# seshnadathur/victor

Measured on AMD Instinct MI355X. Metric: likelihood evals/sec (40 s-bins, 100 mu, l=0,2,4), higher is better.
Workload: dtype f64

## Files before the change

victor_amd/csrc/vk_kernel_cells.h:

```cpp
#pragma once
#include "vk_kernel_fast.h"

namespace vk {

struct CellsPlan {
  int mu, w, s, betar, da, v1, sva, image_end, acc, like, total;
};

__host__ __device__ inline int cells_range_bins(int n_mu, int cpi) { return (cpi + n_mu - 2) / n_mu + 1; }

__host__ __device__ inline CellsPlan make_cells_plan(int n_mu, int n_x, int n_s, int uni_n, int nlr, int n_beta_r,
                                                     int lut_n, int with_da, int cpi, int n_like, int n_sva = 0) {
  CellsPlan p;
  int o = fast_fixed_doubles(uni_n, nlr, lut_n);
  o = (o + 1) & ~1;
  p.mu = o;    o += 2 * n_mu;
  p.w = o;     o += kMaxEll * n_mu;
  p.s = o;     o += (n_s + 1) & ~1;
  p.betar = o; o += (n_beta_r + 1) & ~1;
  p.da = o;    o += with_da ? uni_n * 4 : 0;
  p.v1 = o;    o += with_da == 1 ? 0 : uni_n * 4;
  o = (o + 1) & ~1;
  p.sva = o;   o += (n_sva + 1) & ~1;
  p.image_end = o;
  int bins = cells_range_bins(n_mu, cpi);
  if (bins > n_s) bins = n_s;
  p.acc = o;   o += kMaxEll * (bins + 1) * kWaves;
  o = (o + 1) & ~1;
  p.like = o;  o += n_like > 0 ? like_lds_doubles(n_like) : 0;
  p.total = o;
  return p;
}

template <int NLR>
__device__ __forceinline__ void stage_cells(const TheoryArgs& a, const CellsPlan& pl, double* lds, int with_da) {
  const int tid = threadIdx.x;
  for (int i = tid; i < a.n_mu; i += kBlock) {
    const double m = a.mu[i];
    lds[pl.mu + 2 * i] = m;
    lds[pl.mu + 2 * i + 1] = sqrt(1.0 - m * m);
#pragma unroll
    for (int l = 0; l < kMaxEll; ++l) lds[pl.w + l * a.n_mu + i] = (l < a.n_ell) ? a.w_ell[l * a.n_mu + i] : 0.0;
  }
  for (int j = tid; j < a.n_s; j += kBlock) lds[pl.s + j] = a.s[j];
  stage_uni_records<NLR>(a, lds);
  if (with_da) stage_da<NLR>(a, lds + pl.da);
  if (with_da != 1) for (int e = tid; e < a.uni_n * 4; e += kBlock) lds[pl.v1 + e] = a.uni_sv_v[(e >> 2) * 8 + 4 + (e & 3)];
  if (a.n_beta_r > 0)
    for (int i = tid; i < a.n_beta_r; i += kBlock) lds[pl.betar + i] = a.beta_r[i];
  if (pl.image_end > pl.sva)
    for (int e = tid; e < a.sva_doubles; e += kBlock) lds[pl.sva + e] = a.sva[e];
}

template <int NL>
__device__ __forceinline__ void finish_point_ranges(const TheoryArgs& a, long long point, double beta, double poison, double* th,
                                                    bool gather, const double* lds_beta_r) {
  const int N = a.n_ell * a.n_s;
  const double w0 = a.wsum[0], w1 = a.wsum[1], w2 = a.wsum[2];
  const bool keep_out = !a.fuse || a.want_theory;
  LikePrefetch<kLikeRowsCells> pf;
  if (a.fuse) pf.issue(a.like, beta, late_tid(), lds_beta_r);
  for (int e = late_tid(); gather && e < N; e += kBlock) {
    const int l = (e >= 2 * a.n_s) ? 2 : (e >= a.n_s ? 1 : 0), j = e - l * a.n_s;
    const int q_first = (j * a.n_mu) / a.cells_per_item, q_last = (j * a.n_mu + a.n_mu - 1) / a.cells_per_item;
    double part[8];
    load_shared_x8(partial_slot(a, point, l, j), part);
    double v = 0.0;
#pragma unroll
    for (int c = 0; c < kMaxParts; ++c) v += (c <= q_last - q_first) ? part[c] : 0.0;
    v = v - (l == 0 ? w0 : (l == 1 ? w1 : w2)) + poison;
    if (keep_out) a.out[point * (long long)N + e] = v;
    th[e] = v;
  }
  __syncthreads();
  if (a.fuse) like_point_workgroup(a.like, point, beta, th, th + like_red_off(N), pf);
}

template <int NL>
__device__ __forceinline__ void project_trip(double g, bool first, bool second, const double* w_i, int n_mu, double* acc, int lstride, int lane) {
  const double ga = first ? g : 0.0, gb = second ? g : 0.0;
  double z[NL];
#pragma unroll
  for (int l = 0; l < NL; ++l) {
    const double w = w_i[l * n_mu];
    z[l] = vkm::fold32(w * ga, w * gb);
  }
  double x;
  int l_mine;
  bool mine;
  const int row = lane >> 4;
  if (NL == 3) {
    const double u = vkm::fold16(z[0], z[1]);
    const double v = vkm::fold16(z[2], 0.0);
    const bool up = (lane & 8) != 0;
    const double keep = up ? v : u, send = up ? u : v;
    x = keep + vkm::dpp_move<0x128, 0xF, true>(send);
    l_mine = up ? 2 : (row & 1);
    mine = (lane & 7) == 0 && !(up && (row & 1));
  } else {
    x = vkm::fold16(z[0], NL == 2 ? z[NL - 1] : 0.0);
    x += vkm::dpp_move<0x128, 0xF, true>(x);
    l_mine = row & 1;
    mine = (lane & 15) == 0 && (NL == 2 || !(row & 1));
  }
  x = vkm::octet_sum(x);
  if (mine) acc[l_mine * lstride + (lane >> 5) * kWaves] += x;
}

template <int NLR, int NL, int GRID, int MODE, int SVA = 0>
__global__ __launch_bounds__(kBlock, (MODE == kModeStreaming && !SVA) || MODE == kModeKaiser ? 5 : 4) void vk_theory_cells_kernel(TheoryArgs a) {
  extern __shared__ double lds[];
  vkm::clamp_keeps_nan();
  warm_kernarg_lines<sizeof(TheoryArgs)>();
  const int N = a.n_ell * a.n_s;
  const int R = a.parts;
  const int cpi = a.cells_per_item;
  const bool xi_out = NL == 1 && a.xi_out != 0;
  const bool tail = !xi_out && (a.fuse || R > 1);
  CellsPlan pl = make_cells_plan(a.n_mu, a.n_x, a.n_s, a.uni_n, NLR, a.n_beta_r, a.uni_lut_n, mode_layout(MODE), xi_out ? 0 : cpi,
                                 tail ? N : 0, SVA ? a.sva_doubles : 0);
  pl.like = __builtin_amdgcn_readfirstlane(pl.like);
  const int tid = threadIdx.x;
  VK_STAMP(a, 0);
  if (a.image) copy_image(lds, a.image, pl.image_end);
  else stage_cells<NLR>(a, pl, lds, mode_layout(MODE));
  constexpr bool kHalf = MODE != kModeKaiser;
  const FastConsts fc = make_fast_consts<NLR>(a, kHalf, SVA ? pl.sva : 0);
  __syncthreads();
  VK_STAMP(a, 1);

  const int lane = tid & 63;
  const int wave = __builtin_amdgcn_readfirstlane(tid >> 6);
  const double* l_mu = lds + pl.mu;
  const double* l_w = lds + pl.w;
  const double* l_s = lds + pl.s;
  const int slots = xi_out ? 1 : min(cells_range_bins(a.n_mu, cpi), a.n_s) + 1;
  double* l_acc = lds + pl.acc;
  const unsigned items = (unsigned)a.n * (unsigned)R;
  const int all_cells = a.n_s * a.n_mu;

  {
    const unsigned item = blockIdx.x;
    if (item >= items) return;
    const long long point = item / (unsigned)R;
    const int q = (int)(item - (unsigned)point * (unsigned)R);
    const int c0 = q * cpi, c1 = min(c0 + cpi, all_cells);
    const int jf = (int)__umulhi((unsigned)c0, a.nmu_magic);
    const int nb = (int)__umulhi((unsigned)(c1 - 1), a.nmu_magic) - jf + 1;
    const double* row = a.params + point * VK_NPAR;
    const PointScalars ps = point_scalars(a, row);
    const FastPoint fp = make_fast_point(ps, fc, kHalf);
    constexpr int PV = MODE == kModeKaiser ? 0 : 1;
    __syncthreads();
    rebuild_point_tables<NLR, PV>(a, lds, pl.betar, pl.v1, row[VK_P_BETA], ps.av, mode_is_dispersion(MODE) ? -fp.Gk : fp.AVk,
                                  mode_has_da(MODE) ? lds + pl.da : nullptr);
    if (mode_has_da(MODE) && a.empirical && !a.vr_beta_dep) rebuild_da_emp(a, lds + pl.da, ps.av);
    for (int e = lane; e < kMaxEll * slots; e += 64) l_acc[e * kWaves + wave] = 0.0;
    __syncthreads();
    VK_STAMP(a, 2);
    for (int base = c0 + 64 * wave; base < c1; base += 64 * kWaves) {
      const int e = base + lane;
      const bool live = e < c1;
      const unsigned ec = (unsigned)(live ? e : c1 - 1);
      const int hi = xi_out ? (a.n_s == 1 ? (int)ec : (int)__umulhi(ec, a.ns_magic)) : (int)__umulhi(ec, a.nmu_magic);
      const int lo = (int)ec - hi * (xi_out ? a.n_s : a.n_mu);
      const int j = xi_out ? lo : hi;
      const int i = xi_out ? hi : lo;
      const int jj = j - jf;
      const double sj = l_s[j];
      const vk_d2 mm = *reinterpret_cast<const vk_d2*>(l_mu + 2 * i);
      const double s_perp = sj * fp.k_perp * mm.y;
      const double sperp2 = s_perp * s_perp;
      const double sperp2x = sperp2 * fp.fp2;
      const double s_par = sj * fp.k_par * mm.x;
      double g = 0.0;
      const bool inside = !mode_has_da(MODE) && !__any(!cell_in_table(fc, s_par, sperp2, a.xw_max * fabs(fp.Bk)));
      double gs = 0.0;
      if (MODE == kModeKaiser) {
        g = kaiser_value<NLR, GRID>(lds, lds + pl.da, fc, fp, ps.M, ps.Q, a.niter, a.coord_shift != 0, a.kaiser_approx != 0,
                                    a.rsd == VK_RSD_EUCLID, a.from_data != 0, s_par, sperp2);
      } else if (mode_is_dispersion(MODE)) {
        const double inv_den0 = disp_first_pass<NLR, GRID>(lds, fc, fp, a.niter, s_par, sperp2);
        for (int k = 0; k < a.n_xg; ++k) {
          const VelocityNode xw = load_node(a.xgw, k);
          gs += disp_value<NLR, GRID, MODE == kModeDispersionFromData, SVA>(lds, lds + pl.da, fc, fp, a.niter, fma(-xw.x, fp.Bk, s_par), inv_den0,
                                                                     sperp2, xw.x);
          if (xw.last != 0) {
            asm volatile("" ::: "memory");
            g = fma(xw.w, gs, g);
            gs = 0.0;
          }
        }
      } else if (inside) {
        VelocityNode nxt = load_node(a.xgw, 0);
        for (int k = 0; k < a.n_xg; ++k) {
          const VelocityNode xw = nxt;
          nxt = load_node(a.xgw, k + 1);
          double inv_sv;
          const double p = uni_point<NLR, GRID, MODE == kModeFromData, 1, 0, 0, SVA>(lds, fc, 0.0, fma(-xw.x, fp.Bk, s_par), sperp2, xw.x, fp.fa,
                                                                            sperp2x, 0u, inv_sv);
          gs = fma(inv_sv, p, gs);
          if (xw.last != 0) {
            asm volatile("" ::: "memory");
            g = fma(xw.w, gs, g);
            gs = 0.0;
          }
        }
      } else {
        VelocityNode nxt = load_node(a.xgw, 0);
        for (int k = 0; k < a.n_xg; ++k) {
          const VelocityNode xw = nxt;
          nxt = load_node(a.xgw, k + 1);
          double inv_sv;
          const double p = uni_point<NLR, GRID, MODE == kModeFromData, 1, 1, 0, SVA>(lds, fc, 0.0, fma(-xw.x, fp.Bk, s_par), sperp2, xw.x, fp.fa,
                                                                            sperp2x, 0u, inv_sv);
          gs = fma(inv_sv, p, gs);
          if (xw.last != 0) {
            asm volatile("" ::: "memory");
            g = fma(xw.w, gs, g);
            gs = 0.0;
          }
        }
      }
      if (xi_out) {
        if (live) a.out[point * (long long)all_cells + e] = g - 1.0 + ps.poison;
        continue;
      }
      const int jj0 = __builtin_amdgcn_readfirstlane(jj);
      project_trip<NL>(g, live && jj == jj0, live && jj != jj0, l_w + i, a.n_mu, l_acc + jj0 * kWaves + wave, slots * kWaves, lane);
    }
    if (xi_out) return;
    __syncthreads();
    double* th = lds + pl.like;
    for (int e = late_tid(); e < NL * nb; e += kBlock) {
      const int l = e / nb, jl = e - l * nb;
      const int j = jf + jl;
      const double* pa = l_acc + (l * slots + jl) * kWaves;
      const double sum = (pa[0] + pa[1]) + (pa[2] + pa[3]);
      if (R > 1) {
        store_shared(partial_slot(a, point, l, j) + (q - (j * a.n_mu) / cpi), sum);
      } else {
        const double v = sum - (l == 0 ? a.wsum[0] : (l == 1 ? a.wsum[1] : a.wsum[2])) + ps.poison;
        if (!a.fuse || a.want_theory) a.out[point * (long long)N + l * a.n_s + j] = v;
        if (tail) th[l * a.n_s + j] = v;
      }
    }
    VK_STAMP(a, 3);
    if (tail) {
      bool last = true;
      if (R > 1) {
        int* flag = reinterpret_cast<int*>(th + like_red_off(N) + kLikeRed + 2);
        last = point_completed(a.counters, point, (unsigned)R, flag);
      }
      VK_STAMP(a, 4);
      if (last) {
        finish_point_ranges<NL>(a, point, row[VK_P_BETA], ps.poison, th, R > 1, a.n_beta_r > 0 ? lds + pl.betar : nullptr);
        VK_STAMP(a, 5);
      }
      return;
    }
  }
}


}
```

victor_amd/csrc/victor_hip.hip:

```cpp

#include <hip/hip_runtime.h>
#include <chrono>
#include <cstddef>

#include <cmath>
#include <cstdarg>
#include <cstdio>
#include <cstdlib>
#include <cstring>
#include <limits>
#include <new>
#include <algorithm>
#include <atomic>
#include <map>
#include <string>
#include <vector>

#include "victor_hip.h"
#include "vk_host.h"
#include "vk_ledger.h"
#include "vk_kernel_cells.h"
#include "vk_kernel_fast.h"
#include "vk_kernel_generic.h"
#ifdef VK_DEV_LANES
// ... 841 lines not shown
    ctx->fast_ok = ok;
    ctx->matter_vt = t->matter_model == VK_MATTER_VELOCITY_TEMPLATE;
    ctx->vt_amp = t->vt_amp;
    ctx->matter_lb = t->matter_model == VK_MATTER_LINEAR_BIAS;
    ctx->vr_beta_dep = t->vr_beta_dep ? 1 : 0;
  }
  Uploader up;
  const size_t o_s = up.add(t->s, t->n_s), o_mu = up.add(t->mu, t->n_mu),
               o_w = up.add(t->w_ell, (size_t)t->n_ell * t->n_mu), o_x = up.add(t->x, t->n_x),
               o_wx = up.add(t->w_x, t->n_x);
  const double zero_one[2] = {0.0, 1.0};
  const size_t o_x1 = up.add(zero_one, 2);
  std::vector<double> xw_scaled(2 * ((size_t)t->n_x + 1), 0.0);
  for (int k = 0; k < t->n_x; ++k) {
    xw_scaled[2 * k] = t->x[k] * vkm::kExpScale;
    xw_scaled[2 * k + 1] = t->w_x[k];
    ctx->xw_max = std::max(ctx->xw_max, std::fabs(xw_scaled[2 * k]));
  }
  const size_t o_xws = up.add(xw_scaled.data(), xw_scaled.size());
  std::vector<double> xgw;
  {
    std::vector<char> taken(t->n_x, 0);
    for (int k0 = 0; k0 < t->n_x; ++k0) {
      if (taken[k0] || t->w_x[k0] == 0.0) continue;
      for (int k = k0; k < t->n_x; ++k)
        if (!taken[k] && t->w_x[k] == t->w_x[k0]) {
          taken[k] = 1;
          xgw.push_back(t->x[k] * vkm::kExpScale);
          xgw.push_back(0.0);
        }
      xgw.back() = t->w_x[k0];
    }
    ctx->n_xg = (int)(xgw.size() / 2);
    xgw.resize(xgw.size() + 2, 0.0);
  }
  const size_t o_xgw = up.add(xgw.data(), xgw.size());
  const size_t o_br = t->n_beta_r > 0 ? up.add(t->beta_r, t->n_beta_r) : 0;
  const size_t xi_coef_n = t->n_beta_r > 0 ? (size_t)t->n_ell_r * (t->n_beta_r - 1) * t->xi.n_int * 16
                                           : (size_t)t->n_ell_r * t->xi.n_int * 4;
  const size_t o_xik = up.add(t->xi.knots, t->xi.n_int + 1), o_xic = up.add(t->xi.coef, xi_coef_n);
  const size_t vr_coef_n = t->vr_beta_dep ? (size_t)2 * (t->n_beta_r - 1) * t->vr.n_int * 16 : (size_t)kVrVars * t->vr.n_int * 4;
  const size_t o_vrk = up.add(t->vr.knots, t->vr.n_int + 1), o_vrc = up.add(t->vr.coef, vr_coef_n);
  const bool have_vr_emp = t->vr_beta_dep && t->vr_emp;
  const size_t o_vre = have_vr_emp ? up.add(t->vr_emp, (size_t)3 * (t->n_beta_r - 1) * t->vr.n_int * 28) : 0;
  const size_t o_svk = up.add(t->sv.knots, t->sv.n_int + 1),
               o_svc = up.add(t->sv.coef, t->sv_n_mu ? 4 : (size_t)t->sv.n_int * 4);
  size_t o_svmu = 0, o_sv2d = 0, o_sva = 0;
  if (t->sv_n_mu) {
    o_svmu = up.add(t->sv_mu, t->sv_n_mu);
    o_sv2d = up.add(t->sv2d, (size_t)t->sv.n_int * (t->sv_n_mu - 1) * 16);
    if (ctx->fast_ok) {
      const int nm = t->sv_n_mu - 1;
      const double h = 1.0 / t->sv.inv_h;
      std::vector<double> blk((size_t)t->sv.n_int * nm * 16 + t->sv_n_mu);
      for (size_t e = 0; e < (size_t)t->sv.n_int * nm * 16; ++e) {
        const int pw = (int)((e >> 2) & 3);
        blk[e] = t->sv2d[e] * (pw == 0 ? 1.0 : pw == 1 ? h : pw == 2 ? h * h : h * h * h);
      }
      for (int k = 0; k < t->sv_n_mu; ++k) blk[(size_t)t->sv.n_int * nm * 16 + k] = t->sv_mu[k];
      o_sva = up.add(blk.data(), blk.size());
      ctx->sva_doubles = (int)blk.size();
    }
  }
  size_t o_usv = 0, o_uxi = 0, o_uxc = 0, o_ulut = 0, o_uk = 0, o_uvb = 0, o_uv2 = 0, o_uda = 0, o_uge = 0, o_udab = 0, o_uempb = 0;
  const bool have_lut = t->uni_n > 0 && t->uni_lut_n > 0 && t->uni_lut && t->uni_knots;
  if (have_lut) {
    std::vector<double> packed(((size_t)t->uni_lut_n + 3) / 4, 0.0);
// ... 1108 lines not shown
```

victor_amd/csrc/vk_devmath.h:

```cpp
#pragma once

#include <hip/hip_runtime.h>

namespace vkm {

template <int CTRL, int ROW_MASK, bool BOUND_CTRL = false>
__device__ __forceinline__ double dpp_move(double v) {
  int lo = __double2loint(v), hi = __double2hiint(v);
  lo = __builtin_amdgcn_update_dpp(0, lo, CTRL, ROW_MASK, 0xF, BOUND_CTRL);
  hi = __builtin_amdgcn_update_dpp(0, hi, CTRL, ROW_MASK, 0xF, BOUND_CTRL);
  return __hiloint2double(hi, lo);
}

__device__ __forceinline__ double wave_sum(double v) {
  v += dpp_move<0xB1, 0xF, true>(v);
  v += dpp_move<0x4E, 0xF, true>(v);
  v += dpp_move<0x141, 0xF, true>(v);
  v += dpp_move<0x140, 0xF, true>(v);
  v += dpp_move<0x142, 0xF, true>(v);
  v += dpp_move<0x143, 0xF, true>(v);
  const int lo = __builtin_amdgcn_readlane(__double2loint(v), 63);
  const int hi = __builtin_amdgcn_readlane(__double2hiint(v), 63);
  return __hiloint2double(hi, lo);
}
// ... 45 lines not shown
constexpr int kExpNonposTab = 256;
__device__ __forceinline__ double exp2_frac(int j) { return exp2((double)j * (1.0 / kExpNonposTab)); }

__device__ __forceinline__ double fma3(double p, double f, double c) {
  double r;
  asm("v_fma_f64 %0, %1, %2, %3" : "=v"(r) : "v"(p), "v"(f), "v"(c));
  return r;
}

__device__ __forceinline__ double exp_nonpos(double a, const double* __restrict__ tab) {
  a = fmax(a, -750.0);
  const double n = rint(a * 369.3299304675746);
  double f = fma(n, -0x1.62e42fee00000p-9, a);
  f = fma(n, -0x1.a39ef35793c76p-41, f);
  const int ni = (int)n;
  const double t = tab[ni & (kExpNonposTab - 1)];
  double p = fma3(f, 1.0 / 24.0, 1.0 / 6.0);
  p = fma(p, f, 0.5);
  p = fma(p, f, 1.0);
  p = fma(p, f, 1.0);
  return ldexp(t * p, ni >> 8);
}

__device__ __forceinline__ double fma_s(double p, double f, double c) {
  double r;
  asm("v_fma_f64 %0, %1, %2, %3" : "=v"(r) : "v"(p), "v"(f), "s"(c));
  return r;
}

__device__ __forceinline__ double recip_nr(double x) {
  const double y = __builtin_amdgcn_rcp(x);
  const double e = fma(-x, y, 1.0);
  return fma(y, e, y);
}

__device__ __forceinline__ double rsqrt_nr_x2(double x) {
  const double y = __builtin_amdgcn_rsq(x);
  const double h = x * y;
  const double w = fma(-h, y, 3.0);
  return y * w;
}

__device__ __forceinline__ double rsqrt3_x2(double x) {
  const double y = __builtin_amdgcn_rsq(x);
  const double e = fma(-(x * y), y, 1.0);
  const double p2 = fma(0.75, e, 1.0);
  return y * fma(e, p2, 2.0);
}

constexpr double kExpScale = 13.589148804608305 * 0x1p-9;
constexpr double kExpC = 709.782712893383996843;
template <int EXPT> struct ExpCfg;
template <> struct ExpCfg<0> {
  static constexpr int kBits = 8, kEntries = 256, kDoubles = 256, kDegree = 3;
  static constexpr double kMagic = 0x1.8p34;
  static constexpr double kLead = kExpC * kExpC * kExpC / 6.0;
};
template <> struct ExpCfg<1> {
  static constexpr int kBits = 6, kEntries = 64, kDoubles = 64 * 32, kDegree = 4;
  static constexpr double kMagic = 0x1.8p36;
  static constexpr double kLead = kExpC * kExpC * kExpC * kExpC / 24.0;
};
constexpr int kExpTab = ExpCfg<0>::kDoubles;

template <int EXPT>
__device__ __forceinline__ double exp_table_entry(int j) {
// ... 45 lines not shown
```

victor_amd/csrc/vk_kernel_fast.h:

```cpp
#pragma once
#include "vk_common.h"
#include "vk_kernel_like.h"

namespace vk {

typedef double vk_d2 __attribute__((ext_vector_type(2)));
constexpr int kMuRec = 6;
constexpr int kEtabOff = 0;
template <int EXPT> __host__ __device__ constexpr int recs_off() { return vkm::ExpCfg<EXPT>::kDoubles; }
__host__ __device__ constexpr int recs_off_rt(int expt) { return expt ? vkm::ExpCfg<1>::kDoubles : vkm::ExpCfg<0>::kDoubles; }

__host__ __device__ constexpr int uni_stride(int nlr) { return 4 * (2 + nlr) + 2; }
__host__ __device__ constexpr int fast_fixed_doubles(int uni_n, int nlr, int lut_n, int expt = 0) {
  return recs_off_rt(expt) + (uni_n + (lut_n > 0 ? 2 : 0)) * uni_stride(nlr) + (lut_n + 3) / 4;
}

struct FastConsts {
  double inv_h;
  double off, t_lo, n_eps;
  double inv_g;
  double rlo2, rhi2;
  int lut_off;
  double sv_a, sv_b, sv_tmax;
  double mu_lo, mu_hi, mu_inv_h;
  int sva_off, svmu_off, sv_nm;
};

__device__ __forceinline__ double vmin_f64(double a, double b) {
  double r;
  asm("v_min_f64 %0, %1, %2" : "=v"(r) : "v"(a), "v"(b));
  return r;
}
__device__ __forceinline__ double vmax_f64(double a, double b) {
  double r;
  asm("v_max_f64 %0, %1, %2" : "=v"(r) : "v"(a), "v"(b));
  return r;
}

__device__ __forceinline__ const double* lds_at(const double* base, int byte_off) {
  return reinterpret_cast<const double*>(reinterpret_cast<const char*>(base) + byte_off);
}

__device__ __forceinline__ double cubic_b128(const double* rec, double t) {
  const vk_d2 lo = *reinterpret_cast<const vk_d2*>(rec);
  const vk_d2 hi = *reinterpret_cast<const vk_d2*>(rec + 2);
  return fma(fma(fma(hi.y, t, hi.x), t, lo.y), t, lo.x);
}

template <int NLR, int EXPT = 0>
__device__ __forceinline__ FastConsts make_fast_consts(const TheoryArgs& a, bool half, int sva_off_doubles = 0) {
  FastConsts fc;
  const double sq = half ? 0.25 : 1.0;
  fc.sv_a = fc.sv_b = fc.sv_tmax = fc.mu_lo = fc.mu_hi = fc.mu_inv_h = 0.0;
  fc.sva_off = fc.svmu_off = fc.sv_nm = 0;
  if (a.sv_n_mu > 0 && a.sva_doubles > 0 && a.uni_lut_n == 0) {
    fc.sv_a = a.sv.inv_h / a.uni_inv_h;
    fc.sv_b = -a.sv.knots[0] * a.sv.inv_h;
    fc.sv_tmax = (double)a.sv.n_int * (1.0 - 0x1p-52);
    fc.sv_nm = a.sv_n_mu - 1;
    fc.mu_lo = a.sv_mu[0];
    fc.mu_hi = a.sv_mu[fc.sv_nm];
    fc.mu_inv_h = a.sv_mu_inv_h;
    fc.sva_off = sva_off_doubles * 8;
    fc.svmu_off = (sva_off_doubles + a.sv.n_int * fc.sv_nm * 16) * 8;
  }
  if (a.uni_lut_n > 0) {
    fc.inv_h = 1.0;
    fc.off = 0.0;
    fc.t_lo = a.uni_knots[0];
    fc.n_eps = a.uni_knots[a.uni_n] * (1.0 - 0x1p-52);
    fc.inv_g = a.uni_lut_inv_g;
    fc.rlo2 = sq * fc.t_lo * fc.t_lo * (1.0 + 1e-9);
    fc.rhi2 = sq * fc.n_eps * fc.n_eps * (1.0 - 1e-9);
    fc.lut_off = (recs_off<EXPT>() + (a.uni_n + 2) * uni_stride(NLR)) * 8;
  } else {
    fc.inv_h = a.uni_inv_h;
    fc.off = -a.uni_u0 * a.uni_inv_h;
    fc.t_lo = (a.vr.knots[0] - a.uni_u0) * a.uni_inv_h;
    fc.n_eps = (double)a.uni_n * (1.0 - 0x1p-52);
    fc.inv_g = 0.0;
    const double lo = fc.t_lo - fc.off, hi = fc.n_eps - fc.off;
    fc.rlo2 = sq * lo * lo * (1.0 + 1e-9);
    fc.rhi2 = sq * hi * hi * (1.0 - 1e-9);
    fc.lut_off = 0;
  }
  return fc;
}

__device__ __forceinline__ bool cell_in_table(const FastConsts& fc, double s_par, double sperp2, double xi_max) {
  const double spx = fabs(s_par) + xi_max;
  const double spn = fmax(fabs(s_par) - xi_max, 0.0);
  return (fma(spn, spn, sperp2) >= fc.rlo2) && (fma(spx, spx, sperp2) < fc.rhi2);
}

template <int NLR, int EXPT = 0>
__device__ __forceinline__ void stage_uni_records(const TheoryArgs& a, double* lds) {
  constexpr int stride = uni_stride(NLR);
  double* recs = lds + recs_off<EXPT>();
  const int tid = threadIdx.x;
  for (int e = tid; e < a.uni_n * 8; e += kBlock) recs[(e >> 3) * stride + (e & 7)] = a.uni_sv_v[e];
  if (a.n_beta_r == 0) {
    const double* src = (NLR > 1) ? a.uni_xic : a.uni_xi;
    const int per_l = a.uni_n * 4;
    for (int e = tid; e < NLR * per_l; e += kBlock) {
      const int l = e / per_l, iq = e - l * per_l;
      recs[(iq >> 2) * stride + 8 + 4 * l + (iq & 3)] = src[e];
    }
  }
  const double* etab = EXPT ? a.exp_tab_rep : a.exp_tab;
  for (int j = tid; j < vkm::ExpCfg<EXPT>::kDoubles; j += kBlock) lds[kEtabOff + j] = etab[j];
  if (a.uni_lut_n > 0) {
    for (int q = tid; q <= a.uni_n + 1; q += kBlock) {
      const double left = a.uni_knots[q < a.uni_n ? q : a.uni_n];
      recs[q * stride + stride - 2] = left;
      recs[q * stride + stride - 1] = (q < a.uni_n) ? 1.0 / (a.uni_knots[q + 1] - left) : 0.0;
      if (q >= a.uni_n)
        for (int e = 0; e < stride - 2; ++e) recs[q * stride + e] = 0.0;
    }
    unsigned short* lut = reinterpret_cast<unsigned short*>(recs + (a.uni_n + 2) * stride);
    for (int c = tid; c < a.uni_lut_n; c += kBlock) lut[c] = a.uni_lut[c];
  }
}

__device__ __forceinline__ double poly6(const double* __restrict__ c, double db) {
  double v = c[6];
#pragma unroll
// ... 82 lines not shown
}

struct FastPoint {
  double fa, fp2;
  double Gk, gD;
  double k_perp, k_par;
  double Bk;
  double AVk;
};

__device__ __forceinline__ FastPoint make_fast_point(const PointScalars& ps, const FastConsts& fc, bool half) {
  FastPoint fp;
  const double hs = half ? 0.5 : 1.0;
  const double k = ps.inv_c * fc.inv_h;
  const double kl = k * hs;
  fp.k_perp = ps.aperp * kl;
  fp.k_par = ps.apar * kl;
  fp.Bk = ps.B * kl * (1.0 / vkm::kExpScale);
  fp.AVk = ps.A * vkm::kExpScale * hs;
  const double c = 1.0 / ps.inv_c;
  fp.fa = c * ps.inv_apar;
  fp.fp2 = (c * ps.inv_aperp) * (c * ps.inv_aperp);
  fp.Gk = ps.G * k * (half ? 0.25 : 1.0);
  fp.gD = ps.gD;
  return fp;
}

template <int NLR, int GRID, int CL = 1, int EXPT = 0>
__device__ __forceinline__ const double* locate(const double* __restrict__ lds, const FastConsts& fc, double x,
                                                double& tq, int& qi) {
  constexpr int stride = uni_stride(NLR);
  constexpr int roff = recs_off<EXPT>();
  if (GRID == 0) {
    const double t = CL ? vmin_f64(vmax_f64(x, fc.t_lo), fc.n_eps) : x;
    tq = __builtin_amdgcn_fract(t);
    qi = (int)t;
    return lds_at(lds + roff, __mul24(qi, stride * 8));
  }
  const double u = CL ? vmin_f64(vmax_f64(x, fc.t_lo), fc.n_eps) : x;
  const int cell = (int)(u * fc.inv_g);
  const int q0 = *reinterpret_cast<const unsigned short*>(reinterpret_cast<const char*>(lds) + fc.lut_off + 2 * cell);
  const double* rec0 = lds_at(lds + roff, __mul24(q0, stride * 8));
  const double k1 = rec0[2 * stride - 2], k2 = rec0[3 * stride - 2];
  const int q = q0 + (u >= k1) + (u >= k2);
  qi = q;
  const double* rec = lds_at(lds + roff, __mul24(q, stride * 8));
  const vk_d2 kw = *reinterpret_cast<const vk_d2*>(rec + stride - 2);
  tq = (u - kw.x) * kw.y;
  return rec;
}

__device__ __forceinline__ double sv_aniso(const double* __restrict__ lds, const FastConsts& fc, double rp, double mu2) {
  const double ts = vmin_f64(vmax_f64(fma(rp, fc.sv_a, fc.sv_b), 0.0), fc.sv_tmax);
  const double du = __builtin_amdgcn_fract(ts);
  const int i = (int)ts;
  const double m = vmin_f64(vmax_f64(0.5 * mu2, fc.mu_lo), fc.mu_hi);
  const double* muk = lds_at(lds, fc.svmu_off);
  int j;
  if (fc.mu_inv_h > 0.0) {
    j = min((int)((m - fc.mu_lo) * fc.mu_inv_h), fc.sv_nm - 1);
  } else {
    j = 0;
    for (int k = 1; k < fc.sv_nm; ++k) j += (m >= muk[k]) ? 1 : 0;
  }
  const double dm = m - muk[j];
  const double* c = lds_at(lds, fc.sva_off + (i * fc.sv_nm + j) * 128);
  double acc = cubic_b128(c + 12, dm);
  acc = fma(acc, du, cubic_b128(c + 8, dm));
  acc = fma(acc, du, cubic_b128(c + 4, dm));
  return fma(acc, du, cubic_b128(c, dm));
}

template <int NLR, int GRID, int FD, int PV = 0, int CL = 1, int EXPT = 0, int SVA = 0>
__device__ __forceinline__ double uni_point(const double* __restrict__ lds, const FastConsts& fc, double AVh,
                                            double num, double sperp2, double xk, double fa, double sperp2x,
                                            unsigned lane_off, double& inv_sv) {
  const double X = fma(num, num, sperp2);
  const double yy = vkm::rsqrt_nr_x2(X);
  const double mu2 = num * yy;
  double mu_x = mu2;
  double tq;
  int qi;
  const double rp = SVA ? X * yy : 0.0;
  const double* rec = locate<NLR, GRID, CL, EXPT>(lds, fc, GRID == 0 ? (SVA ? rp + fc.off : fma(X, yy, fc.off)) : X * yy, tq, qi);
  const double SV = SVA ? sv_aniso(lds, fc, rp, mu2) : cubic_b128(rec, tq);
  const double V = cubic_b128(rec + 4, tq);
  const double ynum = PV ? fma(V, mu2, xk) : fma(AVh * V, mu2, xk);
  if (FD) {
    const double rp = num * fa;
    const double Xx = fma(rp, rp, sperp2x);
    const double yyx = vkm::rsqrt_nr_x2(Xx);
    mu_x = rp * yyx;
    rec = locate<NLR, GRID, 1, EXPT>(lds, fc, GRID == 0 ? fma(Xx, yyx, fc.off) : Xx * yyx, tq, qi);
  }
  double xi1 = cubic_b128(rec + 8, tq);
  if (NLR > 1) {
    const double m2 = mu_x * mu_x;
    if (NLR == 2) {
      xi1 = fma(cubic_b128(rec + 12, tq), m2, xi1);
    } else {
      xi1 = fma(fma(cubic_b128(rec + 16, tq), m2, cubic_b128(rec + 12, tq)), m2, xi1);
    }
  }
  inv_sv = vkm::recip_nr(SV);
  const double e = vkm::exp_gauss<EXPT>(ynum, inv_sv, lds + kEtabOff, lane_off);
  return e * xi1;
}

template <int NLR, int GRID>
__device__ __forceinline__ double disp_first_pass(const double* __restrict__ lds, const FastConsts& fc, const FastPoint& fp,
                                                  int niter, double s_par, double sperp2) {
  double tq;
  int qi;
  const bool last = niter == 0;
  const double X = fma(s_par, s_par, sperp2);
  const double yy = last ? vkm::rsqrt3_x2(X) : vkm::rsqrt_nr_x2(X);
  const double* rec = locate<NLR, GRID>(lds, fc, GRID == 0 ? fma(X, yy, fc.off) : X * yy, tq, qi);
  const double den = fma(cubic_b128(rec + 4, tq), yy, 1.0);
  return last ? vkm::recip(den) : vkm::recip_nr(den);
}

template <int NLR, int GRID, int FD, int SVA = 0>
__device__ __forceinline__ double disp_value(const double* __restrict__ lds, const double* __restrict__ da,
                                             const FastConsts& fc, const FastPoint& fp, int niter, double num,
                                             double inv_den0, double sperp2, double xk) {
  double tq;
  int qi;
  auto pass = [&](double rp, bool last) {
    const double X = fma(rp, rp, sperp2);
    const double yy = last ? vkm::rsqrt3_x2(X) : vkm::rsqrt_nr_x2(X);
    const double* rec = locate<NLR, GRID>(lds, fc, GRID == 0 ? fma(X, yy, fc.off) : X * yy, tq, qi);
    const double den = fma(cubic_b128(rec + 4, tq), yy, 1.0);
    return num * (last ? vkm::recip(den) : vkm::recip_nr(den));
  };
  double r_par = num * inv_den0;
  for (int it = __builtin_amdgcn_readfirstlane(niter) - 1; it > 0; --it) r_par = pass(r_par, false);
  if (niter >= 1) r_par = pass(r_par, true);
  const double X = fma(r_par, r_par, sperp2);
  const double yy = vkm::rsqrt3_x2(X);
// ... 371 lines not shown
```

Before: 2.645 million.

## Give each wave a contiguous run of cell trips and accumulate projections per bin

Cells are now split so each wave handles a contiguous run of 64-cell trips instead of interleaving trips across waves. The s-bin and mu indices are tracked incrementally rather than recomputed by magic division. Multipole contributions are accumulated in registers and reduced across lanes only when a trip leaves an s-bin, instead of after every trip. The per-bin accumulator slot count drops by one, the first velocity node is hoisted out of the loop, and the poison value is made wave-uniform. The cost is more complex bookkeeping for trips that straddle bins, and a pending final projection after the loop.

Measured after the change: 2.607 million. 1.4% lower.

```diff
diff --git a/victor_amd/csrc/vk_cells_runs.h b/victor_amd/csrc/vk_cells_runs.h
--- /dev/null
+++ b/victor_amd/csrc/vk_cells_runs.h
@@ -0,0 +1,32 @@
+#pragma once
+
+#if defined(__HIPCC__) || defined(__CUDACC__)
+#define VK_RUNS_HD __host__ __device__
+#else
+#define VK_RUNS_HD
+#endif
+
+namespace vk {
+
+struct CellsRun { int first_trip, trips; };
+VK_RUNS_HD inline CellsRun cells_wave_run(int cells, int wave, int waves) {
+  const int trips = (cells + 63) >> 6;
+  const int q = trips / waves, r = trips - q * waves;
+  CellsRun run;
+  run.first_trip = wave * q + (wave < r ? wave : r);
+  run.trips = q + (wave < r ? 1 : 0);
+  return run;
+}
+
+struct CellsTrip {
+  int j0, i0;
+  VK_RUNS_HD bool whole(int n_mu, int lim) const { return lim >= 63 && i0 + 63 < n_mu; }
+  VK_RUNS_HD bool straddles(int n_mu, int lim) const { return i0 + (lim < 63 ? lim : 63) >= n_mu; }
+  VK_RUNS_HD bool leaves(int n_mu) const { return i0 + 64 >= n_mu; }
+  VK_RUNS_HD void advance(int n_mu) {
+    i0 += 64;
+    if (i0 >= n_mu) { i0 -= n_mu; j0 += 1; }
+  }
+};
+
+}
diff --git a/victor_amd/csrc/vk_kernel_cells.h b/victor_amd/csrc/vk_kernel_cells.h
--- a/victor_amd/csrc/vk_kernel_cells.h
+++ b/victor_amd/csrc/vk_kernel_cells.h
@@ -1,5 +1,6 @@
 #pragma once
 #include "vk_kernel_fast.h"
+#include "vk_cells_runs.h"
 
 namespace vk {
 
@@ -25,7 +26,7 @@
   p.image_end = o;
   int bins = cells_range_bins(n_mu, cpi);
   if (bins > n_s) bins = n_s;
-  p.acc = o;   o += kMaxEll * (bins + 1) * kWaves;
+  p.acc = o;   o += kMaxEll * bins * kWaves;
   o = (o + 1) & ~1;
   p.like = o;  o += n_like > 0 ? like_lds_doubles(n_like) : 0;
   p.total = o;
@@ -77,34 +78,14 @@
 }
 
 template <int NL>
-__device__ __forceinline__ void project_trip(double g, bool first, bool second, const double* w_i, int n_mu, double* acc, int lstride, int lane) {
-  const double ga = first ? g : 0.0, gb = second ? g : 0.0;
-  double z[NL];
-#pragma unroll
-  for (int l = 0; l < NL; ++l) {
-    const double w = w_i[l * n_mu];
-    z[l] = vkm::fold32(w * ga, w * gb);
-  }
-  double x;
-  int l_mine;
-  bool mine;
+__device__ __forceinline__ void project_bin(const double (&z)[NL], double* acc, int lstride, int lane) {
+  const double u = vkm::fold32(z[0], NL >= 2 ? z[NL >= 2 ? 1 : 0] : 0.0);
+  double x = vkm::fold16(u, NL == 3 ? vkm::fold32(z[NL - 1], 0.0) : 0.0);
+  x += vkm::dpp_move<0x128, 0xF, true>(x);
+  x = vkm::octet_sum(x);
   const int row = lane >> 4;
-  if (NL == 3) {
-    const double u = vkm::fold16(z[0], z[1]);
-    const double v = vkm::fold16(z[2], 0.0);
-    const bool up = (lane & 8) != 0;
-    const double keep = up ? v : u, send = up ? u : v;
-    x = keep + vkm::dpp_move<0x128, 0xF, true>(send);
-    l_mine = up ? 2 : (row & 1);
-    mine = (lane & 7) == 0 && !(up && (row & 1));
-  } else {
-    x = vkm::fold16(z[0], NL == 2 ? z[NL - 1] : 0.0);
-    x += vkm::dpp_move<0x128, 0xF, true>(x);
-    l_mine = row & 1;
-    mine = (lane & 15) == 0 && (NL == 2 || !(row & 1));
-  }
-  x = vkm::octet_sum(x);
-  if (mine) acc[l_mine * lstride + (lane >> 5) * kWaves] += x;
+  const bool mine = (lane & 15) == 0 && (row == 0 || (row == 2 && NL >= 2) || (row == 1 && NL == 3));
+  if (mine) acc[(row == 0 ? 0 : 3 - row) * lstride] = x;
 }
 
 template <int NLR, int NL, int GRID, int MODE, int SVA = 0>
@@ -134,7 +115,7 @@
   const double* l_mu = lds + pl.mu;
   const double* l_w = lds + pl.w;
   const double* l_s = lds + pl.s;
-  const int slots = xi_out ? 1 : min(cells_range_bins(a.n_mu, cpi), a.n_s) + 1;
+  const int slots = xi_out ? 1 : min(cells_range_bins(a.n_mu, cpi), a.n_s);
   double* l_acc = lds + pl.acc;
   const unsigned items = (unsigned)a.n * (unsigned)R;
   const int all_cells = a.n_s * a.n_mu;
@@ -150,6 +131,8 @@
     const double* row = a.params + point * VK_NPAR;
     const PointScalars ps = point_scalars(a, row);
     const FastPoint fp = make_fast_point(ps, fc, kHalf);
+    const double poison = __hiloint2double(__builtin_amdgcn_readfirstlane(__double2hiint(ps.poison)),
+                                           __builtin_amdgcn_readfirstlane(__double2loint(ps.poison)));
     constexpr int PV = MODE == kModeKaiser ? 0 : 1;
     __syncthreads();
     rebuild_point_tables<NLR, PV>(a, lds, pl.betar, pl.v1, row[VK_P_BETA], ps.av, mode_is_dispersion(MODE) ? -fp.Gk : fp.AVk,
@@ -158,15 +141,32 @@
     for (int e = lane; e < kMaxEll * slots; e += 64) l_acc[e * kWaves + wave] = 0.0;
     __syncthreads();
     VK_STAMP(a, 2);
-    for (int base = c0 + 64 * wave; base < c1; base += 64 * kWaves) {
-      const int e = base + lane;
-      const bool live = e < c1;
-      const unsigned ec = (unsigned)(live ? e : c1 - 1);
-      const int hi = xi_out ? (a.n_s == 1 ? (int)ec : (int)__umulhi(ec, a.ns_magic)) : (int)__umulhi(ec, a.nmu_magic);
-      const int lo = (int)ec - hi * (xi_out ? a.n_s : a.n_mu);
-      const int j = xi_out ? lo : hi;
-      const int i = xi_out ? hi : lo;
-      const int jj = j - jf;
+    const CellsRun run = cells_wave_run(c1 - c0, wave, kWaves);
+    int base = c0 + 64 * run.first_trip;
+    CellsTrip trip;
+    trip.j0 = (int)__umulhi((unsigned)base, a.nmu_magic);
+    trip.i0 = base - trip.j0 * a.n_mu;
+    const VelocityNode node0 = load_node(a.xgw, 0);
+    double z[NL];
+#pragma unroll
+    for (int l = 0; l < NL; ++l) z[l] = 0.0;
+    bool pending = false;
+    for (int t = 0; t < run.trips; ++t, base += 64) {
+      const int lim = c1 - 1 - base;
+      const int lc = min(lane, lim);
+      const bool live = lane <= lim;
+      const int e = base + lc;
+      int j, i;
+      bool wrap = false;
+      if (xi_out) {
+        i = a.n_s == 1 ? e : (int)__umulhi((unsigned)e, a.ns_magic);
+        j = e - i * a.n_s;
+      } else {
+        i = trip.i0 + lc;
+        wrap = i >= a.n_mu;
+        j = trip.j0 + (wrap ? 1 : 0);
+        i -= wrap ? a.n_mu : 0;
+      }
       const double sj = l_s[j];
       const vk_d2 mm = *reinterpret_cast<const vk_d2*>(l_mu + 2 * i);
       const double s_perp = sj * fp.k_perp * mm.y;
@@ -192,7 +192,7 @@
           }
         }
       } else if (inside) {
-        VelocityNode nxt = load_node(a.xgw, 0);
+        VelocityNode nxt = node0;
         for (int k = 0; k < a.n_xg; ++k) {
           const VelocityNode xw = nxt;
           nxt = load_node(a.xgw, k + 1);
@@ -207,7 +207,7 @@
           }
         }
       } else {
-        VelocityNode nxt = load_node(a.xgw, 0);
+        VelocityNode nxt = node0;
         for (int k = 0; k < a.n_xg; ++k) {
           const VelocityNode xw = nxt;
           nxt = load_node(a.xgw, k + 1);
@@ -223,13 +223,34 @@
         }
       }
       if (xi_out) {
-        if (live) a.out[point * (long long)all_cells + e] = g - 1.0 + ps.poison;
+        if (live) a.out[point * (long long)all_cells + e] = g - 1.0 + poison;
         continue;
       }
-      const int jj0 = __builtin_amdgcn_readfirstlane(jj);
-      project_trip<NL>(g, live && jj == jj0, live && jj != jj0, l_w + i, a.n_mu, l_acc + jj0 * kWaves + wave, slots * kWaves, lane);
+      double* acc = l_acc + (trip.j0 - jf) * kWaves + wave;
+      double w[NL];
+#pragma unroll
+      for (int l = 0; l < NL; ++l) w[l] = l_w[l * a.n_mu + i];
+      if (trip.whole(a.n_mu, lim)) {
+#pragma unroll
+        for (int l = 0; l < NL; ++l) z[l] = fma(w[l], g, z[l]);
+        if (trip.leaves(a.n_mu) || t == run.trips - 1) {
+          project_bin<NL>(z, acc, slots * kWaves, lane);
+#pragma unroll
+          for (int l = 0; l < NL; ++l) z[l] = 0.0;
+        }
+      } else {
+        const double ga = live && !wrap ? g : 0.0, gb = live && wrap ? g : 0.0;
+#pragma unroll
+        for (int l = 0; l < NL; ++l) z[l] = fma(w[l], ga, z[l]);
+        project_bin<NL>(z, acc, slots * kWaves, lane);
+#pragma unroll
+        for (int l = 0; l < NL; ++l) z[l] = w[l] * gb;
+      }
+      pending = trip.straddles(a.n_mu, lim);
+      trip.advance(a.n_mu);
     }
     if (xi_out) return;
+    if (pending) project_bin<NL>(z, l_acc + (trip.j0 - jf) * kWaves + wave, slots * kWaves, lane);
     __syncthreads();
     double* th = lds + pl.like;
     for (int e = late_tid(); e < NL * nb; e += kBlock) {
@@ -240,7 +261,7 @@
       if (R > 1) {
         store_shared(partial_slot(a, point, l, j) + (q - (j * a.n_mu) / cpi), sum);
       } else {
-        const double v = sum - (l == 0 ? a.wsum[0] : (l == 1 ? a.wsum[1] : a.wsum[2])) + ps.poison;
+        const double v = sum - (l == 0 ? a.wsum[0] : (l == 1 ? a.wsum[1] : a.wsum[2])) + poison;
         if (!a.fuse || a.want_theory) a.out[point * (long long)N + l * a.n_s + j] = v;
         if (tail) th[l * a.n_s + j] = v;
       }
@@ -254,7 +275,7 @@
       }
       VK_STAMP(a, 4);
       if (last) {
-        finish_point_ranges<NL>(a, point, row[VK_P_BETA], ps.poison, th, R > 1, a.n_beta_r > 0 ? lds + pl.betar : nullptr);
+        finish_point_ranges<NL>(a, point, row[VK_P_BETA], poison, th, R > 1, a.n_beta_r > 0 ? lds + pl.betar : nullptr);
         VK_STAMP(a, 5);
       }
       return;
```

## Batch velocity nodes in blocks of four with shared reciprocal and scalarized constants

Applied to the files above, without the earlier changes.

The streaming velocity-integral loop now processes quadrature nodes four at a time. It splits each point into a head (table lookups) and a tail (Gaussian exp), and computes the four 1/SV reciprocals from a single rcp of their product (Montgomery trick). Per-point and per-table constants are forced into scalar registers via readfirstlane, and the clamp uses SGPR operands, to reduce VGPR pressure and VALU work. The node array padding grows to allow lookahead loads for the block. This costs extra multiplies, adds overflow/underflow risk in the product of four SV values, and raises register pressure from the wider unrolled block.

After: 2.872 million before, 2.927 million after (median of 6 runs). +1.9%, better.

```diff
diff --git a/victor_amd/csrc/victor_hip.hip b/victor_amd/csrc/victor_hip.hip
--- a/victor_amd/csrc/victor_hip.hip
+++ b/victor_amd/csrc/victor_hip.hip
@@ -897,7 +897,7 @@
       xgw.back() = t->w_x[k0];
     }
     ctx->n_xg = (int)(xgw.size() / 2);
-    xgw.resize(xgw.size() + 2, 0.0);
+    xgw.resize(xgw.size() + 8, 0.0);
   }
   const size_t o_xgw = up.add(xgw.data(), xgw.size());
   const size_t o_br = t->n_beta_r > 0 ? up.add(t->beta_r, t->n_beta_r) : 0;
diff --git a/victor_amd/csrc/vk_devmath.h b/victor_amd/csrc/vk_devmath.h
--- a/victor_amd/csrc/vk_devmath.h
+++ b/victor_amd/csrc/vk_devmath.h
@@ -101,6 +101,33 @@
   const double y = __builtin_amdgcn_rcp(x);
   const double e = fma(-x, y, 1.0);
   return fma(y, e, y);
+}
+
+__device__ __forceinline__ void recip_shared2(double a, double b, double& ra, double& rb) {
+  const double P = a * b;
+  const double y = recip(P);
+  ra = y * b;
+  rb = y * a;
+}
+__device__ __forceinline__ void recip_shared3(double a, double b, double c, double& ra, double& rb, double& rc) {
+  const double ab = a * b;
+  const double P = ab * c;
+  const double y = recip(P);
+  const double yc = y * c;
+  rc = y * ab;
+  ra = yc * b;
+  rb = yc * a;
+}
+__device__ __forceinline__ void recip_shared4(double a, double b, double c, double d, double& ra, double& rb, double& rc, double& rd) {
+  const double ab = a * b, cd = c * d;
+  const double P = ab * cd;
+  const double y = recip(P);
+  const double yab = y * ab;
+  const double ycd = y * cd;
+  ra = ycd * b;
+  rb = ycd * a;
+  rc = yab * d;
+  rd = yab * c;
 }
 
 __device__ __forceinline__ double rsqrt_nr_x2(double x) {
diff --git a/victor_amd/csrc/vk_kernel_cells.h b/victor_amd/csrc/vk_kernel_cells.h
--- a/victor_amd/csrc/vk_kernel_cells.h
+++ b/victor_amd/csrc/vk_kernel_cells.h
@@ -76,6 +76,10 @@
   if (a.fuse) like_point_workgroup(a.like, point, beta, th, th + like_red_off(N), pf);
 }
 
+__device__ __forceinline__ double uniform_f64(double v) {
+  return __hiloint2double(__builtin_amdgcn_readfirstlane(__double2hiint(v)), __builtin_amdgcn_readfirstlane(__double2loint(v)));
+}
+
 template <int NL>
 __device__ __forceinline__ void project_trip(double g, bool first, bool second, const double* w_i, int n_mu, double* acc, int lstride, int lane) {
   const double ga = first ? g : 0.0, gb = second ? g : 0.0;
@@ -105,6 +109,62 @@
   }
   x = vkm::octet_sum(x);
   if (mine) acc[l_mine * lstride + (lane >> 5) * kWaves] += x;
+}
+
+constexpr int kNodeBlock = 4;
+
+template <int W, int NLR, int GRID, int FD, int CL, int SVA>
+__device__ __forceinline__ void stream_block(const double* __restrict__ lds, const FastConsts& fc, const FastPoint& fp, double s_par,
+                                             double sperp2, double sperp2x, const VelocityNode (&c)[kNodeBlock], double& g, double& gs) {
+  UniHead h[W];
+  double inv[W], p[W];
+#pragma unroll
+  for (int i = 0; i < W; ++i) {
+    h[i] = uni_point_head<NLR, GRID, FD, 1, CL, 0, SVA>(lds, fc, 0.0, fma(-c[i].x, fp.Bk, s_par), sperp2, c[i].x, fp.fa, sperp2x);
+    asm volatile("" : "+v"(h[i].SV), "+v"(h[i].ynum), "+v"(h[i].xi1));
+    __builtin_amdgcn_sched_barrier(0);
+  }
+  if (W == 4) vkm::recip_shared4(h[0].SV, h[1 % W].SV, h[2 % W].SV, h[3 % W].SV, inv[0], inv[1 % W], inv[2 % W], inv[3 % W]);
+  if (W == 3) vkm::recip_shared3(h[0].SV, h[1 % W].SV, h[2 % W].SV, inv[0], inv[1 % W], inv[2 % W]);
+  if (W == 2) vkm::recip_shared2(h[0].SV, h[1 % W].SV, inv[0], inv[1 % W]);
+  if (W == 1) inv[0] = vkm::recip_nr(h[0].SV);
+#pragma unroll
+  for (int i = 0; i < W; ++i) p[i] = uni_point_tail<0>(lds, h[i], inv[i], 0u);
+#pragma unroll
+  for (int i = 0; i < W; ++i) {
+    gs = fma(inv[i], p[i], gs);
+    if (c[i].last != 0) {
+      asm volatile("" ::: "memory");
+      g = fma(c[i].w, gs, g);
+      gs = 0.0;
+    }
+  }
+}
+
+template <int NLR, int GRID, int FD, int CL, int SVA>
+__device__ __forceinline__ double stream_cell(const TheoryArgs& a, const double* __restrict__ lds, const FastConsts& fc, const FastPoint& fp,
+                                              double s_par, double sperp2, double sperp2x) {
+  constexpr int W = kNodeBlock;
+  double g = 0.0, gs = 0.0;
+  const double* xgw = a.xgw;
+  asm volatile("" : "+s"(xgw));
+  VelocityNode nx[W];
+#pragma unroll
+  for (int i = 0; i < W; ++i) nx[i] = load_node(xgw, i);
+  const int quads = a.n_xg / W;
+  for (int b = 0; b < quads; ++b) {
+    VelocityNode c[W];
+#pragma unroll
+    for (int i = 0; i < W; ++i) c[i] = nx[i];
+#pragma unroll
+    for (int i = 0; i < W; ++i) nx[i] = load_node(xgw, W * b + W + i);
+    stream_block<W, NLR, GRID, FD, CL, SVA>(lds, fc, fp, s_par, sperp2, sperp2x, c, g, gs);
+  }
+  const int rest = a.n_xg - quads * W;
+  if (rest == 3) stream_block<3, NLR, GRID, FD, CL, SVA>(lds, fc, fp, s_par, sperp2, sperp2x, nx, g, gs);
+  else if (rest == 2) stream_block<2, NLR, GRID, FD, CL, SVA>(lds, fc, fp, s_par, sperp2, sperp2x, nx, g, gs);
+  else if (rest == 1) stream_block<1, NLR, GRID, FD, CL, SVA>(lds, fc, fp, s_par, sperp2, sperp2x, nx, g, gs);
+  return g;
 }
 
 template <int NLR, int NL, int GRID, int MODE, int SVA = 0>
@@ -148,8 +208,22 @@
     const int jf = (int)__umulhi((unsigned)c0, a.nmu_magic);
     const int nb = (int)__umulhi((unsigned)(c1 - 1), a.nmu_magic) - jf + 1;
     const double* row = a.params + point * VK_NPAR;
-    const PointScalars ps = point_scalars(a, row);
-    const FastPoint fp = make_fast_point(ps, fc, kHalf);
+    constexpr bool kStream = !mode_has_da(MODE);
+    PointScalars ps = point_scalars(a, row);
+    if (kStream) ps.poison = uniform_f64(ps.poison);
+    FastPoint fp = make_fast_point(ps, fc, kHalf);
+    if (kStream) {
+      fp.k_perp = uniform_f64(fp.k_perp);
+      fp.k_par = uniform_f64(fp.k_par);
+    }
+    const double xi_max = kStream ? uniform_f64(a.xw_max * fabs(fp.Bk)) : 0.0;
+    const double rlo2 = kStream ? uniform_f64(fc.rlo2) : 0.0, rhi2 = kStream ? uniform_f64(fc.rhi2) : 0.0;
+    FastConsts fcs = fc;
+    if (kStream && GRID == 0) {
+      fcs.off = uniform_f64(fc.off);
+      fcs.t_lo = uniform_f64(fc.t_lo);
+      fcs.n_eps = uniform_f64(fc.n_eps);
+    }
     constexpr int PV = MODE == kModeKaiser ? 0 : 1;
     __syncthreads();
     rebuild_point_tables<NLR, PV>(a, lds, pl.betar, pl.v1, row[VK_P_BETA], ps.av, mode_is_dispersion(MODE) ? -fp.Gk : fp.AVk,
@@ -159,22 +233,25 @@
     __syncthreads();
     VK_STAMP(a, 2);
     for (int base = c0 + 64 * wave; base < c1; base += 64 * kWaves) {
-      const int e = base + lane;
-      const bool live = e < c1;
-      const unsigned ec = (unsigned)(live ? e : c1 - 1);
-      const int hi = xi_out ? (a.n_s == 1 ? (int)ec : (int)__umulhi(ec, a.ns_magic)) : (int)__umulhi(ec, a.nmu_magic);
-      const int lo = (int)ec - hi * (xi_out ? a.n_s : a.n_mu);
-      const int j = xi_out ? lo : hi;
-      const int i = xi_out ? hi : lo;
-      const int jj = j - jf;
+      auto cell_of = [&](int e_, bool& live_, int& i_, int& j_) {
+        live_ = e_ < c1;
+        const unsigned ec = (unsigned)(live_ ? e_ : c1 - 1);
+        const int hi = xi_out ? (a.n_s == 1 ? (int)ec : (int)__umulhi(ec, a.ns_magic)) : (int)__umulhi(ec, a.nmu_magic);
+        const int lo = (int)ec - hi * (xi_out ? a.n_s : a.n_mu);
+        j_ = xi_out ? lo : hi;
+        i_ = xi_out ? hi : lo;
+      };
+      int i0, j;
+      bool live0;
+      cell_of(base + lane, live0, i0, j);
       const double sj = l_s[j];
-      const vk_d2 mm = *reinterpret_cast<const vk_d2*>(l_mu + 2 * i);
+      const vk_d2 mm = *reinterpret_cast<const vk_d2*>(l_mu + 2 * i0);
       const double s_perp = sj * fp.k_perp * mm.y;
       const double sperp2 = s_perp * s_perp;
       const double sperp2x = sperp2 * fp.fp2;
       const double s_par = sj * fp.k_par * mm.x;
       double g = 0.0;
-      const bool inside = !mode_has_da(MODE) && !__any(!cell_in_table(fc, s_par, sperp2, a.xw_max * fabs(fp.Bk)));
+      const bool inside = kStream && !__any(!cell_in_table(rlo2, rhi2, s_par, sperp2, xi_max));
       double gs = 0.0;
       if (MODE == kModeKaiser) {
         g = kaiser_value<NLR, GRID>(lds, lds + pl.da, fc, fp, ps.M, ps.Q, a.niter, a.coord_shift != 0, a.kaiser_approx != 0,
@@ -192,42 +269,22 @@
           }
         }
       } else if (inside) {
-        VelocityNode nxt = load_node(a.xgw, 0);
-        for (int k = 0; k < a.n_xg; ++k) {
-          const VelocityNode xw = nxt;
-          nxt = load_node(a.xgw, k + 1);
-          double inv_sv;
-          const double p = uni_point<NLR, GRID, MODE == kModeFromData, 1, 0, 0, SVA>(lds, fc, 0.0, fma(-xw.x, fp.Bk, s_par), sperp2, xw.x, fp.fa,
-                                                                            sperp2x, 0u, inv_sv);
-          gs = fma(inv_sv, p, gs);
-          if (xw.last != 0) {
-            asm volatile("" ::: "memory");
-            g = fma(xw.w, gs, g);
-            gs = 0.0;
-          }
-        }
+        g = stream_cell<NLR, GRID, MODE == kModeFromData, 0, SVA>(a, lds, fcs, fp, s_par, sperp2, sperp2x);
       } else {
-        VelocityNode nxt = load_node(a.xgw, 0);
-        for (int k = 0; k < a.n_xg; ++k) {
-          const VelocityNode xw = nxt;
-          nxt = load_node(a.xgw, k + 1);
-          double inv_sv;
-          const double p = uni_point<NLR, GRID, MODE == kModeFromData, 1, 1, 0, SVA>(lds, fc, 0.0, fma(-xw.x, fp.Bk, s_par), sperp2, xw.x, fp.fa,
-                                                                            sperp2x, 0u, inv_sv);
-          gs = fma(inv_sv, p, gs);
-          if (xw.last != 0) {
-            asm volatile("" ::: "memory");
-            g = fma(xw.w, gs, g);
-            gs = 0.0;
-          }
-        }
-      }
+        g = stream_cell<NLR, GRID, MODE == kModeFromData, GRID == 0 ? 2 : 1, SVA>(a, lds, fcs, fp, s_par, sperp2, sperp2x);
+      }
+      const int lane2 = kStream ? late_tid() & 63 : lane;
+      const int e = base + lane2;
+      int i = i0, j2 = j;
+      bool live = live0;
+      if (kStream) cell_of(e, live, i, j2);
       if (xi_out) {
         if (live) a.out[point * (long long)all_cells + e] = g - 1.0 + ps.poison;
         continue;
       }
+      const int jj = j2 - jf;
       const int jj0 = __builtin_amdgcn_readfirstlane(jj);
-      project_trip<NL>(g, live && jj == jj0, live && jj != jj0, l_w + i, a.n_mu, l_acc + jj0 * kWaves + wave, slots * kWaves, lane);
+      project_trip<NL>(g, live && jj == jj0, live && jj != jj0, l_w + i, a.n_mu, l_acc + jj0 * kWaves + wave, slots * kWaves, lane2);
     }
     if (xi_out) return;
     __syncthreads();
diff --git a/victor_amd/csrc/vk_kernel_fast.h b/victor_amd/csrc/vk_kernel_fast.h
--- a/victor_amd/csrc/vk_kernel_fast.h
+++ b/victor_amd/csrc/vk_kernel_fast.h
@@ -34,6 +34,17 @@
 __device__ __forceinline__ double vmax_f64(double a, double b) {
   double r;
   asm("v_max_f64 %0, %1, %2" : "=v"(r) : "v"(a), "v"(b));
+  return r;
+}
+
+__device__ __forceinline__ double vmin_f64_s(double a, double b) {
+  double r;
+  asm("v_min_f64 %0, %1, %2" : "=v"(r) : "v"(a), "s"(b));
+  return r;
+}
+__device__ __forceinline__ double vmax_f64_s(double a, double b) {
+  double r;
+  asm("v_max_f64 %0, %1, %2" : "=v"(r) : "v"(a), "s"(b));
   return r;
 }
 
@@ -92,6 +103,11 @@
   const double spn = fmax(fabs(s_par) - xi_max, 0.0);
   return (fma(spn, spn, sperp2) >= fc.rlo2) && (fma(spx, spx, sperp2) < fc.rhi2);
 }
+__device__ __forceinline__ bool cell_in_table(double rlo2, double rhi2, double s_par, double sperp2, double xi_max) {
+  const double spx = fabs(s_par) + xi_max;
+  const double spn = fmax(fabs(s_par) - xi_max, 0.0);
+  return (fma(spn, spn, sperp2) >= rlo2) && (fma(spx, spx, sperp2) < rhi2);
+}
 
 template <int NLR, int EXPT = 0>
 __device__ __forceinline__ void stage_uni_records(const TheoryArgs& a, double* lds) {
@@ -240,7 +256,7 @@
   constexpr int stride = uni_stride(NLR);
   constexpr int roff = recs_off<EXPT>();
   if (GRID == 0) {
-    const double t = CL ? vmin_f64(vmax_f64(x, fc.t_lo), fc.n_eps) : x;
+    const double t = CL == 2 ? vmin_f64_s(vmax_f64_s(x, fc.t_lo), fc.n_eps) : (CL ? vmin_f64(vmax_f64(x, fc.t_lo), fc.n_eps) : x);
     tq = __builtin_amdgcn_fract(t);
     qi = (int)t;
     return lds_at(lds + roff, __mul24(qi, stride * 8));
@@ -279,10 +295,11 @@
   return fma(acc, du, cubic_b128(c, dm));
 }
 
+struct UniHead { double SV, ynum, xi1; };
+
 template <int NLR, int GRID, int FD, int PV = 0, int CL = 1, int EXPT = 0, int SVA = 0>
-__device__ __forceinline__ double uni_point(const double* __restrict__ lds, const FastConsts& fc, double AVh,
-                                            double num, double sperp2, double xk, double fa, double sperp2x,
-                                            unsigned lane_off, double& inv_sv) {
+__device__ __forceinline__ UniHead uni_point_head(const double* __restrict__ lds, const FastConsts& fc, double AVh,
+                                                  double num, double sperp2, double xk, double fa, double sperp2x) {
   const double X = fma(num, num, sperp2);
   const double yy = vkm::rsqrt_nr_x2(X);
   const double mu2 = num * yy;
@@ -299,7 +316,7 @@
     const double Xx = fma(rp, rp, sperp2x);
     const double yyx = vkm::rsqrt_nr_x2(Xx);
     mu_x = rp * yyx;
-    rec = locate<NLR, GRID, 1, EXPT>(lds, fc, GRID == 0 ? fma(Xx, yyx, fc.off) : Xx * yyx, tq, qi);
+    rec = locate<NLR, GRID, CL == 2 ? 2 : 1, EXPT>(lds, fc, GRID == 0 ? fma(Xx, yyx, fc.off) : Xx * yyx, tq, qi);
   }
   double xi1 = cubic_b128(rec + 8, tq);
   if (NLR > 1) {
@@ -310,9 +327,26 @@
       xi1 = fma(fma(cubic_b128(rec + 16, tq), m2, cubic_b128(rec + 12, tq)), m2, xi1);
     }
   }
-  inv_sv = vkm::recip_nr(SV);
-  const double e = vkm::exp_gauss<EXPT>(ynum, inv_sv, lds + kEtabOff, lane_off);
-  return e * xi1;
+  UniHead h;
+  h.SV = SV;
+  h.ynum = ynum;
+  h.xi1 = xi1;
+  return h;
+}
+
+template <int EXPT = 0>
+__device__ __forceinline__ double uni_point_tail(const double* __restrict__ lds, const UniHead& h, double inv_sv, unsigned lane_off) {
+  const double e = vkm::exp_gauss<EXPT>(h.ynum, inv_sv, lds + kEtabOff, lane_off);
+  return e * h.xi1;
+}
+
+template <int NLR, int GRID, int FD, int PV = 0, int CL = 1, int EXPT = 0, int SVA = 0>
+__device__ __forceinline__ double uni_point(const double* __restrict__ lds, const FastConsts& fc, double AVh,
+                                            double num, double sperp2, double xk, double fa, double sperp2x,
+                                            unsigned lane_off, double& inv_sv) {
+  const UniHead h = uni_point_head<NLR, GRID, FD, PV, CL, EXPT, SVA>(lds, fc, AVh, num, sperp2, xk, fa, sperp2x);
+  inv_sv = vkm::recip_nr(h.SV);
+  return uni_point_tail<EXPT>(lds, h, inv_sv, lane_off);
 }
 
 template <int NLR, int GRID>
```
